# VinAIResearch/Point-Unet

Hardware: AMD Instinct MI355X
Metric: points_per_sec_forward (higher is better)
Workload: dtype f32

## Files before the change

point-unet_amd/csrc/att32_tile_walk.h:

```cpp
const int per_xcd = ((((a.n_total + 7) >> 3) + PPT - 1) / PPT) * PPT;
const int xcd = blockIdx.x & 7, slot = blockIdx.x >> 3, slots = gridDim.x >> 3;
const int t_end = min(a.n_total, (xcd + 1) * per_xcd);
const int t_first = xcd * per_xcd + (slot * TPW + tiw) * PPT, t_step = slots * TPW * PPT;
int n_pp[PPT], n_nl = 0;
float n_c[3], n_n[3];
const bool one_cloud = a.n_total == a.n_cloud;
auto cloud_base = [&](int row) { return one_cloud ? 0 : (row / a.n_cloud) * a.n_cloud; };
auto gstage = [&](int st, int t0n) {
    if (t0n >= t_end) return;
    if (st == 0) {
#pragma unroll
        for (int i = 0; i < PPT; ++i) {
            const int t = min(t0n + i, t_end - 1);
            n_pp[i] = a.order ? cloud_base(t) + a.order[t] : t;
        }
    } else if (st == 1) {
        const unsigned p = PPT == 2 ? (c32 >= KN ? n_pp[PPT - 1] : n_pp[0]) : n_pp[0];
        n_nl = a.idx[p * (unsigned)KN + (unsigned)(c32 & (KN - 1))];
        const float* cp = a.xyz + 3u * p;
        n_c[0] = cp[0]; n_c[1] = cp[1]; n_c[2] = cp[2];
    } else {
        const int p = PPT == 2 ? (c32 >= KN ? n_pp[PPT - 1] : n_pp[0]) : n_pp[0];
        n_nl += cloud_base(p);
        const float* np = a.xyz + 3u * (unsigned)n_nl;
        n_n[0] = np[0]; n_n[1] = np[1]; n_n[2] = np[2];
    }
};
gstage(0, t_first);
gstage(1, t_first);
gstage(2, t_first);
```

point-unet_amd/csrc/attpool32b.hip:

```cpp
#include "att32_tile.h"
#include "b3_ops.h"

namespace ps {

struct Att32bArgs : Att32ArgsT<uint4> {};

__device__ __forceinline__ B3Planes load_planes(const uint4* img, int slot, int lane)
{
    B3Planes r;
    r.p[0] = img[(slot * 3 + 0) * 64 + lane];
    r.p[1] = img[(slot * 3 + 1) * 64 + lane];
    r.p[2] = img[(slot * 3 + 2) * 64 + lane];
    return r;
}

template <int D, int STAGE, int KN, int WAVES>
__global__ __launch_bounds__(WAVES * 64) void att32b_kernel(Att32bArgs a)
{
    constexpr int H = D / 2, LDF = H + D, PITCH = H + 4, PPT = 32 / KN;
    constexpr int CBH = H / 32, CBD = D / 32, NQ = H / 16;
    constexpr int W1Q = CBH * 3 * 64, W2Q = STAGE == 2 ? CBH * NQ * 3 * 64 : 0, WBQ = CBD * NQ * 3 * 64;
    constexpr int TILE = 32 * PITCH;
    static_assert(H % 32 == 0 && (KN == 16 || KN == 32), "att32b: d_out >= 64, K in {16, 32}");

    extern __shared__ __attribute__((aligned(16))) float smem[];
    const int wave = __builtin_amdgcn_readfirstlane(threadIdx.x >> 6), lane = threadIdx.x & 63;
    const int hl = lane >> 5, c32 = lane & 31;
    uint4* Wq = reinterpret_cast<uint4*>(smem);
    constexpr int WTOT = (W1Q + W2Q + WBQ) * 4 + 2 * H;
    float* own = smem + WTOT + wave * (32 + TILE);
    int* NB = reinterpret_cast<int*>(own);
    float* T1 = own + 32;
    for (int i = threadIdx.x; i < W1Q; i += WAVES * 64) Wq[i] = a.w1[i];
    for (int i = threadIdx.x; i < W2Q; i += WAVES * 64) Wq[W1Q + i] = a.w2[i];
    for (int i = threadIdx.x; i < WBQ; i += WAVES * 64) Wq[W1Q + W2Q + i] = a.wb[i];
    float* bias = smem + (W1Q + W2Q + WBQ) * 4;
    for (int i = threadIdx.x; i < H; i += WAVES * 64) {
        bias[i] = a.b1[i];
        bias[H + i] = STAGE == 2 ? a.b2[i] : 0.f;
    }
    __syncthreads();
    const uint4 *w1 = Wq, *w2 = Wq + W1Q, *wb = Wq + W1Q + W2Q;
    const float *b1 = bias, *b2 = bias + H;

    constexpr int TPW = WAVES;
    const int tiw = wave;
#include "att32_tile_walk.h"
    for (int t0 = t_first; t0 < t_end; t0 += t_step) {
#include "att32_tile_row.h"
        const float ev[8] = ATT32_LOCSE_K16(enc);
        const B3Planes E = b3_split8<3>(ev);
        if (hl == 0) NB[c32] = nbr;
        gstage(0, t0 + t_step);
        wave_lds_sync();
        unsigned off[16];
        ATT32_ROW_OFFSETS(off, NB, LDF, (unsigned)c32 * 4u);
        const char* fgb = reinterpret_cast<const char*>(a.fg);
        f32x2 gq[2][8], v[2][8];
        auto gather = [&](int i, f32x2 (&gdst)[8], f32x2 (&vdst)[8]) {
            const int rel = i * 32 * 4;
#pragma unroll
            for (int r = 0; r < 16; ++r) gdst[r >> 1][r & 1] = *reinterpret_cast<const float*>(fgb + off[r] + (rel + H * 4));
            if (i * 32 < H) {
#pragma unroll
                for (int r = 0; r < 16; ++r) vdst[r >> 1][r & 1] = *reinterpret_cast<const float*>(fgb + off[r] + rel);
            }
        };
        gather(0, gq[0], v[0]);

        f32x16 f1[CBH];
#pragma unroll
        for (int cb = 0; cb < CBH; ++cb) {
            f32x16 acc;
            ATT32_BIAS_SEED(acc, b1, cb);
            acc = b3_mfma6<3>(load_planes(w1, cb, lane), E, acc);
#pragma unroll
            for (int r = 0; r < 16; ++r) f1[cb][r] = leaky02(acc[r]);
        }
        gstage(1, t0 + t_step);
        B3Planes P[NQ];
        auto split_block = [&](const f32x16& f, B3Planes& lo, B3Planes& hi) {
            const float x0[8] = {f[0], f[1], f[2], f[3], f[4], f[5], f[6], f[7]};
            const float x1[8] = {f[8], f[9], f[10], f[11], f[12], f[13], f[14], f[15]};
            lo = b3_split8<3>(x0);
            hi = b3_split8<3>(x1);
        };
        auto store_block = [&](const f32x16& f, int cb) {
            ATT32_STORE_BLOCK(T1 + c32 * PITCH, cb, , f);
        };
#pragma unroll
        for (int cb = 0; cb < CBH; ++cb) split_block(f1[cb], P[2 * cb], P[2 * cb + 1]);
        if constexpr (STAGE == 1) {
#pragma unroll
            for (int cb = 0; cb < CBH; ++cb) store_block(f1[cb], cb);
        } else {
            f32x16 f2[CBH];
#pragma unroll
            for (int cb = 0; cb < CBH; ++cb) {
                f32x16 acc;
                ATT32_BIAS_SEED(acc, b2, cb);
#pragma unroll
                for (int q = 0; q < NQ; ++q) acc = b3_mfma6<3>(load_planes(w2, cb * NQ + q, lane), P[q], acc);
#pragma unroll
                for (int r = 0; r < 16; ++r) f2[cb][r] = leaky02(acc[r]);
            }
#pragma unroll
            for (int cb = 0; cb < CBH; ++cb) {
                split_block(f2[cb], P[2 * cb], P[2 * cb + 1]);
                store_block(f2[cb], cb);
            }
        }
        wave_lds_sync();
        const float* TX = T1;

#pragma unroll
        for (int cb = 0; cb < CBD; ++cb) {
            if (cb + 1 < CBD) gather(cb + 1, gq[(cb + 1) & 1], v[(cb + 1) & 1]);
            if (cb == 0) gstage(2, t0 + t_step);
            f32x16 acc;
#pragma unroll
            for (int r = 0; r < 16; ++r) acc[r] = 0.f;
#pragma unroll
            for (int q = 0; q < NQ; ++q) acc = b3_mfma6<3>(P[q], load_planes(wb, cb * NQ + q, lane), acc);
            f32x2 (&vv)[8] = v[cb & 1];
            const f32x2 (&gs)[8] = gq[cb & 1];
#include "att32_tile_pool.h"
        }
        wave_lds_sync();
    }
}


template <int D, int STAGE, int KN, int WAVES>
__global__ __launch_bounds__(WAVES * 64) void att32s_kernel(Att32bArgs a)
{
    constexpr int H = D / 2, LDF = H + D, PITCH = H + 4, PPT = 32 / KN;
    constexpr int CBH = H / 32, CBD = D / 32, NQ = H / 16;
    constexpr int PLQ = NQ * 3 * 64;
    constexpr int NB_H = CBH / WAVES, NB_D = CBD / WAVES;
    static_assert(CBH % WAVES == 0 && NB_D == 2 && (KN == 16 || KN == 32), "att32s: two score blocks per wave");

    extern __shared__ __attribute__((aligned(16))) float smem[];
    const int wave = threadIdx.x >> 6, lane = threadIdx.x & 63;
    const int hl = lane >> 5, c32 = lane & 31;
    int* NB = reinterpret_cast<int*>(smem);
    uint4* PA = reinterpret_cast<uint4*>(smem + 32);
    uint4* PB = STAGE == 2 ? PA + PLQ : PA;
    float* TX = reinterpret_cast<float*>(PB + PLQ);

    constexpr int TPW = 1;
    const int tiw = 0;
#include "att32_tile_walk.h"
    auto seed = [&](const float* b, int cb) {
        f32x16 acc;
        ATT32_BIAS_SEED(acc, b, cb);
        return acc;
    };
    auto emit_block = [&](const f32x16& acc, int cb, uint4* planes, bool values) {
        float x0[8], x1[8];
#pragma unroll
        for (int r = 0; r < 8; ++r) { x0[r] = leaky02(acc[r]); x1[r] = leaky02(acc[8 + r]); }
        const B3Planes lo = b3_split8<3>(x0), hi = b3_split8<3>(x1);
#pragma unroll
        for (int pl = 0; pl < 3; ++pl) {
            planes[((2 * cb) * 3 + pl) * 64 + lane] = lo.p[pl];
            planes[((2 * cb + 1) * 3 + pl) * 64 + lane] = hi.p[pl];
        }
        if (values) {
#pragma unroll
            for (int g4 = 0; g4 < 4; ++g4) {
                const float* x = g4 < 2 ? x0 + 4 * g4 : x1 + 4 * (g4 - 2);
                *reinterpret_cast<float4*>(TX + c32 * PITCH + cb * 32 + g4 * 8 + hl * 4) = make_float4(x[0], x[1], x[2], x[3]);
            }
        }
    };
    static_assert(NB_H == 1, "att32s: one transposed block per wave");
    const B3Planes W1 = load_planes(a.w1, wave, lane);
    const f32x16 seed1 = seed(a.b1, wave);
    constexpr int PD = D >= 512 ? 4 : 2;
    constexpr int PD2 = STAGE == 2 ? (D >= 512 ? 4 : 8) : 1;
    const int cbA = wave, cbB = wave + WAVES;
    for (int t0 = t_first; t0 < t_end; t0 += t_step) {
#include "att32_tile_row.h"
        const float ev[8] = ATT32_LOCSE_K16(enc);
        const B3Planes E = b3_split8<3>(ev);
        if (hl == 0 && wave == 0) NB[c32] = nbr;
        gstage(0, t0 + t_step);
        B3Planes ring[PD2], rA[PD], rB[PD];
        if constexpr (STAGE == 2) {
#pragma unroll
            for (int q = 0; q < PD2; ++q) ring[q] = load_planes(a.w2, wave * NQ + q, lane);
        } else {
#pragma unroll
            for (int q = 0; q < PD; ++q) {
                rA[q] = load_planes(a.wb, cbA * NQ + q, lane);
                rB[q] = load_planes(a.wb, cbB * NQ + q, lane);
            }
        }

        emit_block(b3_mfma6<3>(W1, E, seed1), wave, PA, STAGE == 1);
        __syncthreads();
        gstage(1, t0 + t_step);
        unsigned off[16];
        ATT32_ROW_OFFSETS(off, NB, LDF, (unsigned)(wave * 32 + c32) * 4u);
        const char* fgb = reinterpret_cast<const char*>(a.fg);
        if constexpr (STAGE == 2) {
            const int cb = wave;
            f32x16 acc = seed(a.b2, cb);
#pragma unroll 1
            for (int q0 = 0; q0 + PD2 < NQ; q0 += PD2) {
#pragma unroll
                for (int j = 0; j < PD2; ++j) {
                    acc = b3_mfma6<3>(ring[j], load_planes(PA, q0 + j, lane), acc);
                    ring[j] = load_planes(a.w2, cb * NQ + q0 + j + PD2, lane);
                }
            }
#pragma unroll
            for (int j = 0; j < PD2; ++j) acc = b3_mfma6<3>(ring[j], load_planes(PA, NQ - PD2 + j, lane), acc);
#pragma unroll
            for (int q = 0; q < PD; ++q) {
                rA[q] = load_planes(a.wb, cbA * NQ + q, lane);
                rB[q] = load_planes(a.wb, cbB * NQ + q, lane);
            }
            emit_block(acc, cb, PB, true);
            __syncthreads();
        }
        gstage(2, t0 + t_step);

        f32x16 accA, accB;
#pragma unroll
        for (int r = 0; r < 16; ++r) { accA[r] = 0.f; accB[r] = 0.f; }
        f32x2 gq[2][8], v[2][8];
        {
#pragma unroll 1
            for (int q0 = 0; q0 + PD < NQ; q0 += PD) {
#pragma unroll
                for (int j = 0; j < PD; ++j) {
                    const B3Planes x = load_planes(PB, q0 + j, lane);
                    accA = b3_mfma6<3>(x, rA[j], accA);
                    accB = b3_mfma6<3>(x, rB[j], accB);
                    rA[j] = load_planes(a.wb, cbA * NQ + q0 + j + PD, lane);
                    rB[j] = load_planes(a.wb, cbB * NQ + q0 + j + PD, lane);
                }
            }
#pragma unroll
            for (int i = 0; i < 2; ++i)
#pragma unroll
                for (int r = 0; r < 16; ++r) gq[i][r >> 1][r & 1] = *reinterpret_cast<const float*>(fgb + off[r] + (i * WAVES * 32 * 4 + H * 4));
#pragma unroll
            for (int j = 0; j < PD; ++j) {
                const B3Planes x = load_planes(PB, NQ - PD + j, lane);
                accA = b3_mfma6<3>(x, rA[j], accA);
                accB = b3_mfma6<3>(x, rB[j], accB);
            }
        }
#pragma unroll
        for (int r = 0; r < 16; ++r) v[0][r >> 1][r & 1] = *reinterpret_cast<const float*>(fgb + off[r]);
#pragma unroll
        for (int ii = 0; ii < 2; ++ii) {
            const int i = 1 - ii;
            const int cb = wave + i * WAVES;
            const f32x16& acc = i == 0 ? accA : accB;
            f32x2 (&vv)[8] = v[i];
            const f32x2 (&gs)[8] = gq[i];
#include "att32_tile_pool.h"
        }
        __syncthreads();
    }
}

static inline int kmap(int q, int g, int j)
{
    const int r = 8 * (q & 1) + j;
    return 32 * (q >> 1) + (r & 3) + 8 * (r >> 2) + 4 * g;
}

void pack_b3(const float* W, int cin, int cout, uint16_t* out)
{
    const int nq = cin / 16, cbs = cout / 32;
    for (int cb = 0; cb < cbs; ++cb)
        for (int q = 0; q < nq; ++q)
            for (int pl = 0; pl < 3; ++pl)
                for (int l = 0; l < 64; ++l)
                    for (int j = 0; j < 8; ++j)
                        out[(((((size_t)cb * nq + q) * 3 + pl) * 64 + l) * 8) + j] = b3_piece_of(W[(size_t)kmap(q, l >> 5, j) * cout + 32 * cb + (l & 31)], pl);
}

void pack_b3_locse(const float* W1, int cout, uint16_t* out)
{
    const int cbs = cout / 32;
    for (int cb = 0; cb < cbs; ++cb)
        for (int pl = 0; pl < 3; ++pl)
            for (int l = 0; l < 64; ++l)
                for (int j = 0; j < 8; ++j) {
                    const int k = 8 * (l >> 5) + j;
                    out[((((size_t)cb * 3 + pl) * 64 + l) * 8) + j] = k < 10 ? b3_piece_of(W1[(size_t)k * cout + 32 * cb + (l & 31)], pl) : (uint16_t)0;
                }
}

template <int D, int STAGE, int KN>
static int launch_att32b(ps_context* c, const Att32bArgs& a)
{
    constexpr int H = D / 2, PITCH = H + 4, TILE = 32 * PITCH;
    constexpr int CBH = H / 32, CBD = D / 32, NQ = H / 16;
    constexpr int WAVES = D == 128 ? 8 : (STAGE == 1 ? 16 : 12);
    constexpr int PER_CU = 1;
    constexpr size_t planes = (size_t)(CBH + (STAGE == 2 ? CBH * NQ : 0) + CBD * NQ) * 3 * 64 * 16;
    constexpr size_t smem = planes + sizeof(float) * (2 * H + (size_t)WAVES * (32 + TILE));
    static_assert(smem <= 160 * 1024, "att32b: weights + tiles exceed the LDS");
    auto kern = att32b_kernel<D, STAGE, KN, WAVES>;
    PS_HIP(hipFuncSetAttribute(reinterpret_cast<const void*>(kern), hipFuncAttributeMaxDynamicSharedMemorySize, (int)smem));
    const int tiles = ceil_div(a.n_total, 32 / KN);
    const int blocks = (std::min(ceil_div(tiles, WAVES), 256 * PER_CU) + 7) & ~7;
    hipLaunchKernelGGL(kern, dim3(blocks), dim3(WAVES * 64), smem, c->stream, a);
    PS_HIP(hipGetLastError());
    return PS_OK;
}

template <int D, int STAGE, int KN>
static int launch_att32s(ps_context* c, const Att32bArgs& a)
{
    constexpr int H = D / 2, PITCH = H + 4, NQ = H / 16;
    constexpr int WAVES = D / 64;
    constexpr size_t smem = sizeof(float) * 32 + (size_t)(STAGE == 2 ? 2 : 1) * NQ * 3 * 64 * 16 + sizeof(float) * 32 * PITCH;
    static_assert(smem <= 160 * 1024, "att32s: planes + value tile exceed the LDS");
    auto kern = att32s_kernel<D, STAGE, KN, WAVES>;
    if (smem > 48 * 1024) PS_HIP(hipFuncSetAttribute(reinterpret_cast<const void*>(kern), hipFuncAttributeMaxDynamicSharedMemorySize, (int)smem));
    const int tiles = ceil_div(a.n_total, 32 / KN);
    const int blocks = (std::min(tiles, 256 * 16) + 7) & ~7;
    hipLaunchKernelGGL(kern, dim3(blocks), dim3(WAVES * 64), smem, c->stream, a);
    PS_HIP(hipGetLastError());
    return PS_OK;
}

bool att_pool32b_fits(const AttStage& s)
{
    return att_pool32_fits(s) && s.p32->w1b && (s.d == 64 || s.d == 128 || s.d == 256 || s.d == 512);
}

int att_pool32b_stage(ps_context* c, const AttStage& s)
{
    if (s.n_total <= 0) return PS_OK;
    const Att32bArgs a = att32_args<Att32bArgs>(s, s.p32->w1b, s.p32->w2b, s.p32->wb1b, s.p32->wb2b);
    if (s.d == 64) return att32_stage_k(s, [&](auto stage, auto k) { return launch_att32b<64, stage(), k()>(c, a); });
    if (s.d == 128) return att32_stage_k(s, [&](auto stage, auto k) { return launch_att32b<128, stage(), k()>(c, a); });
    if (s.d == 256) return att32_stage_k(s, [&](auto stage, auto k) { return launch_att32s<256, stage(), k()>(c, a); });
    return att32_stage_k(s, [&](auto stage, auto k) { return launch_att32s<512, stage(), k()>(c, a); });
}

}
```

point-unet_amd/csrc/debug_hooks.h:

```cpp
#ifndef POINTSEG_DEBUG_H
#define POINTSEG_DEBUG_H
#include "../../include/pointseg.h"
#ifdef __cplusplus
extern "C" {
#endif
int ps_debug_knn_host(const float* support, const float* queries, int64_t B, int64_t n_support,
                      int64_t n_queries, int64_t K, int32_t* out_idx);
int ps_debug_kdtree_host(const float* support, int64_t n, int32_t* vind, int32_t* nodes, float* pts,
                         int32_t* root_depth, float* bbox);
int ps_debug_kdtree_device(ps_context* ctx, const float* support, int64_t n, int32_t* vind, int32_t* nodes,
                           float* pts, int32_t* root_depth, float* bbox);
#define PS_DEBUG_KDTREE_STATS 22
int ps_debug_kdtree_device_set(ps_context* ctx, const float* support, const int32_t* n, int64_t T, const int32_t* want_copy, int32_t* vind,
                               int32_t* nodes, float* pts, int32_t* fat, int32_t* root_depth, float* bbox, float* copy, int32_t* stats);
int ps_debug_pack_weights(const float* W, int cin, int cout, int ntb, float* out);
int ps_debug_pack_b3(const float* W, int cin, int cout, uint16_t* out);
int ps_debug_gemm32(ps_context* ctx, int split_bf16, const float* x1, int ld1, int c1, const int32_t* g1, const float* x2, int ld2, int c2,
                    const int32_t* g2, int gm, int gn, const float* W, const float* bias, int64_t R, int cout, int leaky, float* y, int ldy);
int ps_debug_gemm32_plan(ps_context* ctx, int split_bf16, int64_t R, int cin, int cout, int* out4);

typedef struct ps_debug_chain_layer {
    const float* W;
    const float* bias;
    int cin, cout, leaky;
    float* y;
    int ldy;
    const float* extra;
    int ld_extra, c_extra;
    const int32_t* extra_gather;
} ps_debug_chain_layer;
typedef struct ps_debug_chain_desc {
    int n_layers;
    ps_debug_chain_layer layer[4];
    const float* x1; const int32_t* g1; int ld1, c1, g1m, g1n;
    const float* x2; const int32_t* g2; int ld2, c2, g2m, g2n;
    int64_t R;
} ps_debug_chain_desc;
int ps_debug_chain(ps_context* ctx, const ps_debug_chain_desc* d, int form);
int ps_debug_chain_plan(const ps_debug_chain_desc* d, int* out4);
int ps_debug_set_regchain_b3(ps_context* ctx, int on);
int ps_debug_set_att_lane(ps_context* ctx, int on);
int ps_debug_att_stage(ps_randla* net, int level, int stage, int form, const float* xyz, const int32_t* idx, const int32_t* order, const float* fg,
                       int64_t n_total, int64_t n_cloud, float* agg);
int ps_debug_att_form(ps_randla* net, int level, int stage, int k, int64_t n_total);
int ps_debug_att_lane_pass_points(void);

int ps_debug_set_tuning(ps_context* ctx, const char* field, double value);
int ps_debug_get_tuning(ps_context* ctx, const char* field, double* value);
int ps_debug_tuning_fields(char* buf, int cap);
int ps_debug_volume_sample_args_size(void);

int64_t ps_debug_scan_words(int64_t n);
int64_t ps_debug_sort_words(int64_t n);
int ps_debug_scan_launches(int64_t n);
int ps_debug_sort_launches(int64_t n, int bits);
int ps_debug_scan_u32(ps_context* ctx, const uint32_t* in, uint32_t* out, int64_t n, uint32_t* work);
int ps_debug_sort_pairs(ps_context* ctx, int key_bytes, void* k0, void* k1, uint32_t* v0, uint32_t* v1, int64_t n, int bits, uint32_t* work,
                        int* which_out);
int ps_debug_reduce_partials(ps_context* ctx, int form, const void* part, int n_part, int nv, int n0, void* out0, void* out1);

#ifdef __cplusplus
}
#endif
#endif
```

point-unet_amd/csrc/debug_hooks.hip:

```cpp
#include "common.h"

#include <cstring>
#include <vector>
#include "kdtree_build.h"
#include "kdtree_host.h"
#include "rowgemm.h"
#include "attpool.h"
#include "debug_hooks.h"
#include "randla_net.h"
#include "reduce_partials.h"
#include "sortscan.h"

using namespace ps;

extern "C" int ps_debug_volume_sample_args_size(void) { return (int)sizeof(ps_volume_sample_args); }

extern "C" int ps_debug_pack_weights(const float* W, int cin, int cout, int ntb, float* out)
{
    PS_CHECK(W && out && (ntb == 1 || ntb == 2 || ntb == 4), "ps_debug_pack_weights: bad argument");
    pack_weights(W, cin, cout, ntb, out);
    return PS_OK;
}

extern "C" int ps_debug_pack_b3(const float* W, int cin, int cout, uint16_t* out)
{
    PS_CHECK(W && out && cin > 0 && cin % 32 == 0 && cout > 0 && cout % 32 == 0, "ps_debug_pack_b3: bad argument");
    pack_b3(W, cin, cout, out);
    return PS_OK;
}

extern "C" int ps_debug_gemm32(ps_context* c, int split_bf16, const float* x1, int ld1, int c1, const int32_t* g1, const float* x2, int ld2, int c2,
                               const int32_t* g2, int gm, int gn, const float* W, const float* bias, int64_t R, int cout, int leaky, float* y, int ldy)
{
    PS_CHECK(c && x1 && W && bias && y && R >= 0 && c1 > 0 && c2 >= 0 && cout > 0, "ps_debug_gemm32: bad argument");
    PS_HIP(hipSetDevice(c->device));
    const int cin = c1 + c2;
    PS_CHECK(cin % (split_bf16 ? 16 : 8) == 0 && cout % 32 == 0, "ps_debug_gemm32: cin %% %d and cout %% 32 must be 0", split_bf16 ? 16 : 8);
    std::vector<float> img((size_t)cin * cout * (split_bf16 ? 3 : 2) / 2);
    if (split_bf16) pack_p32b(W, cin, cout, reinterpret_cast<uint16_t*>(img.data()));
    else pack_p32(W, cin, cout, img.data());
    float *d_img = nullptr, *d_bias = nullptr;
    PS_HIP(hipMalloc(reinterpret_cast<void**>(&d_img), img.size() * sizeof(float)));
    PS_HIP(hipMalloc(reinterpret_cast<void**>(&d_bias), sizeof(float) * (size_t)cout));
    PS_HIP(hipMemcpyAsync(d_img, img.data(), img.size() * sizeof(float), hipMemcpyHostToDevice, c->stream));
    PS_HIP(hipMemcpyAsync(d_bias, bias, sizeof(float) * (size_t)cout, hipMemcpyHostToDevice, c->stream));
    PackedLinear L;
    L.cin = cin; L.cout = cout; L.leaky = leaky; L.bias = d_bias;
    if (split_bf16) L.w32b = d_img; else L.w32 = d_img;
    RowSrc s1, s2;
    s1.x = x1; s1.ld = ld1; s1.c = c1; s1.gather = g1; s1.gm = g1 ? gm : 0; s1.gn = g1 ? gn : 0;
    s2.x = x2; s2.ld = ld2; s2.c = c2; s2.gather = g2; s2.gm = g2 ? gm : 0; s2.gn = g2 ? gn : 0;
    int rc = PS_EINVAL;
    if (split_bf16 ? gemm32b_fits(L, s1, s2, R, ldy) : gemm32_fits(L, s1, s2, R, ldy))
        rc = split_bf16 ? gemm32b(c, L, s1, s2, R, y, ldy) : gemm32(c, L, s1, s2, R, y, ldy);
    else
        set_error("ps_debug_gemm32: the shape does not fit the kernel");
    (void)hipStreamSynchronize(c->stream);
    (void)hipFree(d_img);
    (void)hipFree(d_bias);
    return rc;
}

extern "C" int ps_debug_gemm32_plan(ps_context* c, int split_bf16, int64_t R, int cin, int cout, int* out4)
{
    PS_CHECK(c && out4 && R >= 1 && cin > 0 && cout > 0 && cin % (split_bf16 ? 16 : 8) == 0 && cout % 32 == 0, "ps_debug_gemm32_plan: bad argument");
    const Gemm32Plan p = split_bf16 ? gemm32b_plan(c->tune, R, cin, cout) : gemm32_plan(c->tune, R, cin, cout);
    out4[0] = p.rw;
    out4[1] = p.cw;
    out4[2] = p.sk;
    out4[3] = p.pd;
    return PS_OK;
}

namespace {

struct ChainBuild {
    PackedLinear L[kChainMaxSteps];
    ChainStep steps[kChainMaxSteps];
    RowSrc s1, s2;
    int n = 0;
};

int chain_describe(const ps_debug_chain_desc* d, ChainBuild& b, const float* image)
{
    PS_CHECK(d && d->n_layers >= 1 && d->n_layers <= kChainMaxSteps, "ps_debug_chain: 1..%d layers", kChainMaxSteps);
    PS_CHECK(d->R >= 0 && d->c1 > 0 && d->c2 >= 0 && d->ld1 >= d->c1 && (d->c2 == 0 || d->ld2 >= d->c2), "ps_debug_chain: bad row sources");
    b.n = d->n_layers;
    b.s1.x = d->x1; b.s1.gather = d->g1; b.s1.ld = d->ld1; b.s1.c = d->c1; b.s1.gm = d->g1 ? d->g1m : 0; b.s1.gn = d->g1 ? d->g1n : 0;
    if (d->c2) {
        b.s2.x = d->x2; b.s2.gather = d->g2; b.s2.ld = d->ld2; b.s2.c = d->c2; b.s2.gm = d->g2 ? d->g2m : 0; b.s2.gn = d->g2 ? d->g2n : 0;
    }
    for (int i = 0; i < b.n; ++i) {
        const ps_debug_chain_layer& y = d->layer[i];
        PS_CHECK(y.cin > 0 && y.cout > 0 && y.cin <= 4096 && y.cout <= 4096, "ps_debug_chain: layer %d: bad channel counts", i);
        PS_CHECK(!y.y || y.ldy >= y.cout, "ps_debug_chain: layer %d: ldy below cout", i);
        PS_CHECK(!y.extra || (i > 0 && y.c_extra > 0 && y.ld_extra >= y.c_extra), "ps_debug_chain: layer %d: bad extra source", i);
        PackedLinear& L = b.L[i];
        L = PackedLinear();
        L.cin = y.cin; L.cout = y.cout; L.leaky = y.leaky;
        L.ks = (y.cin + 3) / 4;
        L.ntb = choose_ntb(y.cout);
        L.cblocks = (y.cout + 16 * L.ntb - 1) / (16 * L.ntb);
        L.wp = image; L.bias = image;
        ChainStep& st = b.steps[i];
        st = ChainStep();
        st.L = &L; st.y = y.y; st.ldy = y.ldy;
        if (y.extra) {
            st.extra.x = y.extra; st.extra.ld = y.ld_extra; st.extra.c = y.c_extra; st.extra.gather = y.extra_gather;
        }
    }
    return PS_OK;
}

}

extern "C" int ps_debug_chain_plan(const ps_debug_chain_desc* d, int* out4)
{
    PS_CHECK(d && out4 && d->R >= 1, "ps_debug_chain_plan: bad argument");
    static const float nothing = 0.f;
    ChainBuild b;
    PS_TRY(chain_describe(d, b, &nothing));
    const ChainPlan p = rowchain_plan(b.steps, b.n, b.s1, b.s2, d->R);
    out4[0] = p.form;
    out4[1] = p.form ? p.blocks : 0;
    out4[2] = p.form ? (int)p.lds_bytes : 0;
    out4[3] = p.fast_in;
    return PS_OK;
}

extern "C" int ps_debug_chain(ps_context* c, const ps_debug_chain_desc* d, int form)
{
    PS_CHECK(c && d && form >= 0 && form <= 3, "ps_debug_chain: bad argument");
    ChainBuild b;
    PS_TRY(chain_describe(d, b, nullptr));
    PS_CHECK(d->x1 && (d->c2 == 0 || d->x2), "ps_debug_chain: NULL row source");
    for (int i = 0; i < b.n; ++i) PS_CHECK(d->layer[i].W, "ps_debug_chain: layer %d has no weights", i);
    if (form == 3) {
        int cur = d->c1 + d->c2;
        for (int i = 0; i < b.n; ++i) {
            const ps_debug_chain_layer& y = d->layer[i];
            PS_CHECK(!(y.extra && y.extra_gather), "ps_debug_chain: layer %d: the extra rows of a chain are plain rows", i);
            cur += y.extra ? y.c_extra : 0;
            PS_CHECK(cur == y.cin, "ps_debug_chain: layer %d expects %d channels, the chain gives %d", i, y.cin, cur);
            cur = y.cout;
        }
    }
    if (d->R == 0) return PS_OK;
    PS_HIP(hipSetDevice(c->device));
    std::vector<float> host;
    size_t wp_off[kChainMaxSteps], b_off[kChainMaxSteps], wq_off[kChainMaxSteps], tmp_off[kChainMaxSteps];
    auto grow = [&](size_t floats) {
        const size_t off = (host.size() + 63) & ~size_t(63);
        host.resize(off + floats);
        return off;
    };
    for (int i = 0; i < b.n; ++i) {
        const ps_debug_chain_layer& y = d->layer[i];
        PackedLinear& L = b.L[i];
        wp_off[i] = grow(L.packed_floats());
        pack_weights(y.W, y.cin, y.cout, L.ntb, host.data() + wp_off[i]);
        b_off[i] = grow((size_t)L.cout_pad());
        for (int k = 0; k < L.cout_pad(); ++k) host[b_off[i] + k] = (y.bias && k < y.cout) ? y.bias[k] : 0.f;
        wq_off[i] = 0;
        if (y.cin % 16 == 0) {
            wq_off[i] = grow(L.kperm_floats());
            pack_weights_kperm(y.W, y.cin, y.cout, L.ntb, host.data() + wq_off[i]);
        }
    }
    size_t total = (host.size() + 63) & ~size_t(63);
    for (int i = 0; i < b.n; ++i) {
        tmp_off[i] = total;
        if (form == 3 && !d->layer[i].y) total += ((size_t)d->R * d->layer[i].cout + 63) & ~size_t(63);
    }
    float* dev = nullptr;
    PS_HIP(hipMalloc(reinterpret_cast<void**>(&dev), total * sizeof(float)));
    int rc = PS_OK;
    if (hipMemcpyAsync(dev, host.data(), host.size() * sizeof(float), hipMemcpyHostToDevice, c->stream) != hipSuccess) {
        set_error("ps_debug_chain: upload failed");
        rc = PS_EHIP;
    }
    for (int i = 0; i < b.n; ++i) {
        b.L[i].wp = dev + wp_off[i];
        b.L[i].bias = dev + b_off[i];
        b.L[i].wq = wq_off[i] ? dev + wq_off[i] : nullptr;
    }
    if (rc == PS_OK) {
        if (form == 0) {
            ChainCache cache;
            if (rowchain_fits(b.steps, b.n, b.s1, b.s2)) rc = rowchain(c, b.steps, b.n, b.s1, b.s2, d->R, &cache);
            else { set_error("ps_debug_chain: the chain fits neither chain kernel (channels above %d, mismatched, or a gathered extra)", kChainMaxC); rc = PS_EINVAL; }
            (void)hipStreamSynchronize(c->stream);
            cache.clear();
        } else if (form == 1) {
            if (regchain_fits(b.steps, b.n, b.s1, b.s2)) rc = regchain(c, b.steps, b.n, b.s1, b.s2, d->R, nullptr);
            else { set_error("ps_debug_chain: not one of regchain's compiled chain shapes"); rc = PS_EINVAL; }
        } else if (form == 2) {
            if (rowchain_lds_plan(b.steps, b.n, b.s1, b.s2, d->R).form == 2) rc = rowchain_lds(c, b.steps, b.n, b.s1, b.s2, d->R);
            else { set_error("ps_debug_chain: the chain does not fit the LDS-staged kernel (channels above %d, mismatched, or a gathered extra)", kChainMaxC); rc = PS_EINVAL; }
        } else {
            RowSrc in1 = b.s1, in2 = b.s2;
            for (int i = 0; i < b.n && rc == PS_OK; ++i) {
                const ChainStep& st = b.steps[i];
                if (i > 0) {
                    in2 = RowSrc();
                    if (st.extra.x) in2 = st.extra;
                }
                float* out = st.y ? st.y : dev + tmp_off[i];
                const int ldo = st.y ? st.ldy : b.L[i].cout;
                rc = rowgemm(c, b.L[i], in1, in2, d->R, out, ldo);
                in1 = RowSrc();
                in1.x = out; in1.ld = ldo; in1.c = b.L[i].cout;
            }
        }
    }
    (void)hipStreamSynchronize(c->stream);
    (void)hipFree(dev);
    return rc;
}

extern "C" int ps_debug_set_regchain_b3(ps_context* c, int on)
{
    PS_CHECK(c && (on == 0 || on == 1), "ps_debug_set_regchain_b3: bad argument");
    c->regchain_b3 = on != 0;
    return PS_OK;
}

extern "C" int ps_debug_set_att_lane(ps_context* c, int on)
{
    PS_CHECK(c && (on == 0 || on == 1), "ps_debug_set_att_lane: bad argument");
    c->att_lane = on != 0;
    return PS_OK;
}

extern "C" int ps_debug_att_stage(ps_randla* net, int level, int stage, int form, const float* xyz, const int32_t* idx, const int32_t* order,
                                  const float* fg, int64_t n_total, int64_t n_cloud, float* agg)
{
    PS_CHECK(net && xyz && idx && fg && agg, "ps_debug_att_stage: NULL argument");
    PS_CHECK(net->have_weights, "ps_debug_att_stage: weights not set");
    PS_CHECK(level >= 0 && level < net->cfg.num_layers && (stage == 1 || stage == 2) && form >= 0 && form <= 4, "ps_debug_att_stage: bad level / stage / form");
    PS_CHECK(n_total >= 0 && n_cloud >= 1 && n_total % n_cloud == 0, "ps_debug_att_stage: n_total must be a whole number of clouds");
    ps_context* c = net->ctx;
    PS_HIP(hipSetDevice(c->device));
    const EncLevel& e = net->enc[level];
    const int d = e.d, h = d / 2;
    const bool use_g = d >= 64;
    AttStage s;
    s.xyz = xyz; s.idx = idx; s.order = order; s.fg = fg; s.lfa1 = &e.lfa1; s.agg = agg;
    s.n_total = n_total; s.n_cloud = n_cloud; s.d = d; s.k = net->cfg.k_n; s.ldf = use_g ? h + d : h;
    s.p32 = e.has_p32 ? &e.p32 : nullptr;
    s.lfa2 = stage == 2 ? &e.lfa2 : nullptr;
    s.wbot = use_g ? (stage == 1 ? &e.bot1 : &e.bot2) : nullptr;
    s.wfull = use_g ? nullptr : (stage == 1 ? &e.full1 : &e.full2);
    s.lane = stage == 1 ? e.lane1 : e.lane2;
    int rc = PS_EINVAL;
    if (form == 4) rc = att_lane_stage(c, s);
    else if (form == 0) rc = att_pool_stage(c, s);
    else if (form == 1 && att_pool32b_fits(s)) rc = att_pool32b_stage(c, s);
    else if (form == 2 && att_pool32_fits(s)) rc = att_pool32_stage(c, s);
    else if (form == 3) rc = att_pool16_stage(c, s);
    else set_error("ps_debug_att_stage: the level (d = %d, %lld rows) does not fit the 32x32 form %d", d, (long long)n_total, form);
    (void)hipStreamSynchronize(c->stream);
    return rc;
}

extern "C" int ps_debug_att_form(ps_randla* net, int level, int stage, int k, int64_t n_total)
{
    if (!net || !net->have_weights || level < 0 || level >= net->cfg.num_layers || (stage != 1 && stage != 2) || k < 1 || n_total < 0) {
        set_error("ps_debug_att_form: bad argument");
        return -1;
    }
    const EncLevel& e = net->enc[level];
    const int d = e.d, h = d / 2;
    const bool use_g = d >= 64;
    AttStage s;
    s.lfa1 = &e.lfa1; s.lfa2 = stage == 2 ? &e.lfa2 : nullptr;
    s.wbot = use_g ? (stage == 1 ? &e.bot1 : &e.bot2) : nullptr;
    s.wfull = use_g ? nullptr : (stage == 1 ? &e.full1 : &e.full2);
    s.lane = stage == 1 ? e.lane1 : e.lane2;
    s.p32 = e.has_p32 ? &e.p32 : nullptr;
    s.n_total = n_total; s.n_cloud = n_total; s.d = d; s.k = k; s.ldf = use_g ? h + d : h;
    return att_pool_form(net->ctx, s);
}

extern "C" int ps_debug_att_lane_pass_points(void) { return att_lane_pass_points(); }

static bool is_bool(double v) { return v == 0 || v == 1; }
static bool is_int_in(double v, double lo, double hi) { return v >= lo && v <= hi && v == (double)(int64_t)v; }

#define PS_TUNING_FIELDS(X)                                                \
    X(gemm32b_min_flops, v >= 0 && v <= 1e300)                             \
    X(gemm32b_rw, v == 0 || v == 1 || v == 2)                              \
    X(gemm32b_cw, v == 0 || v == 1 || v == 2)                              \
    X(gemm32_no_sk8, is_bool(v))                                           \
    X(att64_gemm, is_bool(v))                                              \
    X(att64_occ, v == 0 || v == 1 || v == 2)                               \
    X(att_no_split, is_bool(v))                                            \
    X(wgrad_b3_min_rows, is_int_in(v, 0, (double)(1ll << 40)))             \
    X(gemm_b3_min_rows, is_int_in(v, 0, (double)(1ll << 40)))              \
    X(wgrad_wgs, is_int_in(v, 64, 4096))                                   \
    X(bn_slice, is_bool(v))                                                \
    X(inv_bucket, is_bool(v))                                              \
    X(inv_tile, v == 4096 || v == 6144 || v == 8192)                       \
    X(gather_reduce_ordered, is_bool(v))                                   \
    X(maxpool_bwd_ordered, is_bool(v))                                     \
    X(train_act_bf16, is_bool(v))                                          \
    X(train_att_gemm_split, v == -1 || v == 0 || v == 1)                   \
    X(train_att_gemm, is_bool(v))                                          \
    X(train_att128_fwd_gemm, is_bool(v))                                   \
    X(train_fuse_residual, is_bool(v))                                     \
    X(train_merge_syncbn, is_bool(v))                                      \
    X(convbn_max_c, is_int_in(v, 0, 4096))                                 \
    X(convbn_rect_max, is_int_in(v, 0, (double)(1 << 30)))                 \
    X(wgrad_debug, is_bool(v))

extern "C" int ps_debug_set_tuning(ps_context* c, const char* field, double v)
{
    PS_CHECK(c && field, "ps_debug_set_tuning: NULL argument");
#define PS_SET(f, ok)                                                                                 \
    if (std::strcmp(field, #f) == 0) {                                                                \
        PS_CHECK(ok, "ps_debug_set_tuning: %g is not a value %s is compiled for", v, #f);             \
        c->tune.f = static_cast<decltype(c->tune.f)>(v);                                              \
        return PS_OK;                                                                                 \
    }
    PS_TUNING_FIELDS(PS_SET)
#undef PS_SET
    PS_CHECK(false, "ps_debug_set_tuning: no knob named '%s'", field);
}

extern "C" int ps_debug_get_tuning(ps_context* c, const char* field, double* out)
{
    PS_CHECK(c && field && out, "ps_debug_get_tuning: NULL argument");
#define PS_GET(f, ok)                               \
    if (std::strcmp(field, #f) == 0) {              \
        *out = static_cast<double>(c->tune.f);      \
        return PS_OK;                               \
    }
    PS_TUNING_FIELDS(PS_GET)
#undef PS_GET
    PS_CHECK(false, "ps_debug_get_tuning: no knob named '%s'", field);
}

extern "C" int ps_debug_tuning_fields(char* buf, int cap)
{
    static const char names[] =
#define PS_NAME(f, ok) #f "\n"
        PS_TUNING_FIELDS(PS_NAME)
#undef PS_NAME
        ;
    PS_CHECK(buf && cap >= (int)sizeof(names), "ps_debug_tuning_fields: need %d bytes", (int)sizeof(names));
    std::memcpy(buf, names, sizeof(names));
    return PS_OK;
}

extern "C" int ps_debug_kdtree_device(ps_context* c, const float* support, int64_t n, int32_t* vind, int32_t* nodes, float* pts,
                                      int32_t* root_depth, float* bbox)
{
    PS_CHECK(c && support && vind && nodes && pts && root_depth && bbox && n >= 1, "ps_debug_kdtree_device: bad argument");
    PS_HIP(hipSetDevice(c->device));
    PS_TRY(c->stage_in.reserve(sizeof(float) * 3 * (size_t)n));
    PS_HIP(hipMemcpyAsync(c->stage_in.p, support, sizeof(float) * 3 * (size_t)n, hipMemcpyHostToDevice, c->stream));
    TreeSetPlan plan;
    plan.add((int32_t)n);
    for (int pass = 0; pass < 2; ++pass) {
        c->knn_arena.begin(pass == 0);
        plan.carve(c->knn_arena);
        if (pass == 0) PS_TRY(c->knn_arena.buf.reserve(c->knn_arena.off));
    }
    plan.src[0] = c->stage_in.as<float>();
    PS_TRY(build_trees(c, plan));
    int32_t flag[kBuildFlagWords] = {};
    PS_HIP(hipMemcpyAsync(flag, plan.d_flags, sizeof(flag), hipMemcpyDeviceToHost, c->stream));
    PS_HIP(hipStreamSynchronize(c->stream));
    PS_CHECK(flag[kFlagQueueOverflow] == 0, "ps_debug_kdtree_device: builder queue overflow");
    TreeMeta m;
    PS_HIP(hipMemcpyAsync(nodes, plan.d_nodes[0], sizeof(int4) * 2 * (size_t)n, hipMemcpyDeviceToHost, c->stream));
    PS_HIP(hipMemcpyAsync(pts, plan.d_pts[0], sizeof(float4) * (size_t)n, hipMemcpyDeviceToHost, c->stream));
    PS_HIP(hipMemcpyAsync(&m, plan.d_meta, sizeof(TreeMeta), hipMemcpyDeviceToHost, c->stream));
    PS_HIP(hipStreamSynchronize(c->stream));
    for (int64_t i = 0; i < n; ++i) std::memcpy(&vind[i], &pts[4 * i + 3], 4);
    root_depth[0] = m.root;
    root_depth[1] = m.depth;
    for (int a = 0; a < 3; ++a) {
        bbox[a] = m.lo[a];
        bbox[3 + a] = m.hi[a];
    }
    return PS_OK;
}

extern "C" int ps_debug_kdtree_device_set(ps_context* c, const float* support, const int32_t* n, int64_t T, const int32_t* want_copy, int32_t* vind,
                                          int32_t* nodes, float* pts, int32_t* fat, int32_t* root_depth, float* bbox, float* copy, int32_t* stats)
{
    PS_CHECK(c && support && n && T >= 1 && vind && nodes && pts && fat && root_depth && bbox && stats, "ps_debug_kdtree_device_set: bad argument");
    size_t tot = 0, tot_copy = 0;
    for (int64_t i = 0; i < T; ++i) {
        PS_CHECK(n[i] >= 1, "ps_debug_kdtree_device_set: tree %lld has %d points", (long long)i, n[i]);
        tot += (size_t)n[i];
        if (want_copy && want_copy[i]) tot_copy += (size_t)n[i];
    }
    PS_CHECK(tot_copy == 0 || copy, "ps_debug_kdtree_device_set: want_copy without a copy buffer");
    PS_HIP(hipSetDevice(c->device));
    PS_TRY(c->stage_in.reserve(sizeof(float) * 3 * tot));
    PS_HIP(hipMemcpyAsync(c->stage_in.p, support, sizeof(float) * 3 * tot, hipMemcpyHostToDevice, c->stream));
    TreeSetPlan plan;
    for (int64_t i = 0; i < T; ++i) plan.add(n[i]);
    float* d_copy = nullptr;
    for (int pass = 0; pass < 2; ++pass) {
        c->knn_arena.begin(pass == 0);
        plan.carve(c->knn_arena);
        d_copy = c->knn_arena.take<float>(3 * tot_copy + 1);
        if (pass == 0) PS_TRY(c->knn_arena.buf.reserve(c->knn_arena.off));
    }
    plan.copy_dst.assign((size_t)T, nullptr);
    {
        size_t off = 0, off_copy = 0;
        for (int64_t i = 0; i < T; ++i) {
            plan.src[i] = c->stage_in.as<float>() + 3 * off;
            off += (size_t)n[i];
            if (want_copy && want_copy[i]) {
                plan.copy_dst[i] = d_copy + 3 * off_copy;
                off_copy += (size_t)n[i];
            }
        }
    }
    PS_TRY(build_trees(c, plan));
    BuildCounters bc;
    PS_TRY(read_build_counters(c, plan, &bc));
    int32_t flag[kBuildFlagWords] = {};
    PS_HIP(hipMemcpyAsync(flag, plan.d_flags, sizeof(flag), hipMemcpyDeviceToHost, c->stream));
    std::vector<TreeMeta> meta((size_t)T);
    PS_HIP(hipMemcpyAsync(meta.data(), plan.d_meta, sizeof(TreeMeta) * (size_t)T, hipMemcpyDeviceToHost, c->stream));
    {
        size_t off = 0;
        for (int64_t i = 0; i < T; ++i) {
            const size_t ni = (size_t)n[i];
            PS_HIP(hipMemcpyAsync(nodes + 4 * 2 * off, plan.d_nodes[i], sizeof(int4) * 2 * ni, hipMemcpyDeviceToHost, c->stream));
            PS_HIP(hipMemcpyAsync(fat + 4 * 6 * off, plan.d_fat[i], sizeof(int4) * 6 * ni, hipMemcpyDeviceToHost, c->stream));
            PS_HIP(hipMemcpyAsync(pts + 4 * off, plan.d_pts[i], sizeof(float4) * ni, hipMemcpyDeviceToHost, c->stream));
            off += ni;
        }
    }
    if (tot_copy) PS_HIP(hipMemcpyAsync(copy, d_copy, sizeof(float) * 3 * tot_copy, hipMemcpyDeviceToHost, c->stream));
    PS_HIP(hipStreamSynchronize(c->stream));
    for (size_t i = 0; i < tot; ++i) std::memcpy(&vind[i], &pts[4 * i + 3], 4);
    for (int64_t i = 0; i < T; ++i) {
        root_depth[2 * i] = meta[(size_t)i].root;
        root_depth[2 * i + 1] = meta[(size_t)i].depth;
        for (int a = 0; a < 3; ++a) {
            bbox[6 * i + a] = meta[(size_t)i].lo[a];
            bbox[6 * i + 3 + a] = meta[(size_t)i].hi[a];
        }
    }
    static_assert(PS_DEBUG_KDTREE_STATS == 6 + 2 * kBuildCounterLevels, "stats layout (debug_hooks.h)");
    stats[0] = bc.chunked_levels;
    for (int l = 0; l < kBuildCounterLevels; ++l) {
        stats[1 + l] = bc.ntasks[l];
        stats[1 + kBuildCounterLevels + l] = bc.nchunks[l];
    }
    stats[1 + 2 * kBuildCounterLevels] = bc.straggler_tasks;
    stats[2 + 2 * kBuildCounterLevels] = bc.mid_pushed;
    stats[3 + 2 * kBuildCounterLevels] = bc.small_pushed;
    stats[4 + 2 * kBuildCounterLevels] = flag[kFlagStackOverflow];
    stats[5 + 2 * kBuildCounterLevels] = flag[kFlagQueueOverflow];
    return PS_OK;
}

extern "C" int64_t ps_debug_scan_words(int64_t n) { return n < 0 ? -1 : (int64_t)scan_workspace_words((size_t)n); }
extern "C" int64_t ps_debug_sort_words(int64_t n) { return n < 0 ? -1 : (int64_t)sort_workspace_words((size_t)n); }
extern "C" int ps_debug_scan_launches(int64_t n) { return n < 0 ? -1 : scan_launches((size_t)n); }
extern "C" int ps_debug_sort_launches(int64_t n, int bits) { return n < 0 || bits < 1 || bits > 64 ? -1 : radix_sort_pairs_launches((size_t)n, bits); }

extern "C" int ps_debug_scan_u32(ps_context* c, const uint32_t* in, uint32_t* out, int64_t n, uint32_t* work)
{
    PS_CHECK(c && in && out && work && n >= 0, "ps_debug_scan_u32: bad argument");
    PS_HIP(hipSetDevice(c->device));
    exclusive_scan_u32(c->stream, in, out, (size_t)n, work);
    PS_HIP(hipGetLastError());
    PS_HIP(hipStreamSynchronize(c->stream));
    return PS_OK;
}

extern "C" int ps_debug_sort_pairs(ps_context* c, int key_bytes, void* k0, void* k1, uint32_t* v0, uint32_t* v1, int64_t n, int bits, uint32_t* work,
                                   int* which_out)
{
    PS_CHECK(c && k0 && k1 && v0 && v1 && work && which_out && n >= 0, "ps_debug_sort_pairs: bad argument");
    PS_CHECK(key_bytes == 4 || key_bytes == 8, "ps_debug_sort_pairs: key_bytes must be 4 or 8");
    PS_CHECK(bits >= 1 && bits <= 8 * key_bytes, "ps_debug_sort_pairs: bits must be 1..%d", 8 * key_bytes);
    PS_HIP(hipSetDevice(c->device));
    *which_out = key_bytes == 4
                     ? radix_sort_pairs_u32(c->stream, static_cast<unsigned*>(k0), static_cast<unsigned*>(k1), v0, v1, (size_t)n, bits, work)
                     : radix_sort_pairs_u64(c->stream, static_cast<unsigned long long*>(k0), static_cast<unsigned long long*>(k1), v0, v1, (size_t)n,
                                            bits, work);
    PS_HIP(hipGetLastError());
    PS_HIP(hipStreamSynchronize(c->stream));
    return PS_OK;
}

extern "C" int ps_debug_reduce_partials(ps_context* c, int form, const void* part, int n_part, int nv, int n0, void* out0, void* out1)
{
    PS_CHECK(c && part && out0 && n_part >= 0 && nv >= 0 && form >= 0 && form <= 3, "ps_debug_reduce_partials: bad argument");
    PS_CHECK(form < 2 || (out1 && n0 >= 0 && n0 <= nv), "ps_debug_reduce_partials: forms 2 and 3 need out1 and 0 <= n0 <= nv");
    PS_HIP(hipSetDevice(c->device));
    if (nv == 0) return PS_OK;
    const dim3 grid((unsigned)((nv + 15) / 16)), block(256);
    switch (form) {
    case 0:
        hipLaunchKernelGGL(reduce_partials_kernel<float>, grid, block, 0, c->stream, static_cast<const float*>(part), n_part, nv, static_cast<float*>(out0));
        break;
    case 1:
        hipLaunchKernelGGL(reduce_partials_kernel<double>, grid, block, 0, c->stream, static_cast<const double*>(part), n_part, nv,
                           static_cast<double*>(out0));
        break;
    case 2:
        hipLaunchKernelGGL((reduce_partials2_kernel<float>), grid, block, 0, c->stream, static_cast<const float*>(part), n_part, nv, n0,
                           static_cast<float*>(out0), static_cast<float*>(out1));
        break;
    default:
        hipLaunchKernelGGL((reduce_partials2_kernel<float, double>), grid, block, 0, c->stream, static_cast<const float*>(part), n_part, nv, n0,
                           static_cast<float*>(out0), static_cast<float*>(out1));
        break;
    }
    PS_HIP(hipGetLastError());
    PS_HIP(hipStreamSynchronize(c->stream));
    return PS_OK;
}
```

Before: 203.9 million.

## Interleave wave tile walk, batch weight staging loads, use buffer loads for gather

```diff
diff --git a/point-unet_amd/csrc/att32_tile_walk.h b/point-unet_amd/csrc/att32_tile_walk.h
--- a/point-unet_amd/csrc/att32_tile_walk.h
+++ b/point-unet_amd/csrc/att32_tile_walk.h
@@ -1,7 +1,7 @@
 const int per_xcd = ((((a.n_total + 7) >> 3) + PPT - 1) / PPT) * PPT;
 const int xcd = blockIdx.x & 7, slot = blockIdx.x >> 3, slots = gridDim.x >> 3;
 const int t_end = min(a.n_total, (xcd + 1) * per_xcd);
-const int t_first = xcd * per_xcd + (slot * TPW + tiw) * PPT, t_step = slots * TPW * PPT;
+const int t_first = xcd * per_xcd + (tiw * slots + slot) * PPT, t_step = slots * TPW * PPT;
 int n_pp[PPT], n_nl = 0;
 float n_c[3], n_n[3];
 const bool one_cloud = a.n_total == a.n_cloud;
diff --git a/point-unet_amd/csrc/attpool32b.hip b/point-unet_amd/csrc/attpool32b.hip
--- a/point-unet_amd/csrc/attpool32b.hip
+++ b/point-unet_amd/csrc/attpool32b.hip
@@ -4,6 +4,15 @@
 namespace ps {
 
 struct Att32bArgs : Att32ArgsT<uint4> {};
+
+__device__ __forceinline__ __amdgpu_buffer_rsrc_t fg_rsrc(const float* fg, unsigned bytes)
+{
+    return __builtin_amdgcn_make_buffer_rsrc(const_cast<float*>(fg), 0, (int)bytes, 0x00020000);
+}
+__device__ __forceinline__ float fg_load(__amdgpu_buffer_rsrc_t r, unsigned off)
+{
+    return __builtin_bit_cast(float, __builtin_amdgcn_raw_buffer_load_b32(r, (int)off, 0, 0));
+}
 
 __device__ __forceinline__ B3Planes load_planes(const uint4* img, int slot, int lane)
 {
@@ -12,6 +21,23 @@
     r.p[1] = img[(slot * 3 + 1) * 64 + lane];
     r.p[2] = img[(slot * 3 + 2) * 64 + lane];
     return r;
+}
+
+template <int N, int NT, int R>
+__device__ __forceinline__ void stage_load(uint4 (&r)[R], const uint4* __restrict__ src, int tid)
+{
+#pragma unroll
+    for (int j = 0; j * NT < N; ++j) r[j] = src[(j + 1) * NT <= N ? tid + j * NT : min(tid + j * NT, N - 1)];
+}
+template <int N, int NT, bool WHOLE, int R>
+__device__ __forceinline__ void stage_write(uint4* dst, const uint4 (&r)[R], int tid)
+{
+#pragma unroll
+    for (int j = 0; j * NT < N; ++j) {
+        if ((j + 1) * NT <= N) {
+            if (WHOLE) dst[tid + j * NT] = r[j];
+        } else if (!WHOLE && tid + j * NT < N) dst[tid + j * NT] = r[j];
+    }
 }
 
 template <int D, int STAGE, int KN, int WAVES>
@@ -31,9 +57,22 @@
     float* own = smem + WTOT + wave * (32 + TILE);
     int* NB = reinterpret_cast<int*>(own);
     float* T1 = own + 32;
-    for (int i = threadIdx.x; i < W1Q; i += WAVES * 64) Wq[i] = a.w1[i];
-    for (int i = threadIdx.x; i < W2Q; i += WAVES * 64) Wq[W1Q + i] = a.w2[i];
-    for (int i = threadIdx.x; i < WBQ; i += WAVES * 64) Wq[W1Q + W2Q + i] = a.wb[i];
+    {
+        constexpr int NT = WAVES * 64;
+        constexpr int N1 = (W1Q + NT - 1) / NT, N2 = (W2Q + NT - 1) / NT, NB3 = (WBQ + NT - 1) / NT;
+        static_assert(N1 + N2 + NB3 <= 12, "att32b: the staging loads of a thread are held in registers");
+        const int tid = threadIdx.x;
+        uint4 r1[N1], r2[N2 ? N2 : 1], rb[NB3];
+        stage_load<W1Q, NT>(r1, a.w1, tid);
+        stage_load<W2Q, NT>(r2, a.w2, tid);
+        stage_load<WBQ, NT>(rb, a.wb, tid);
+        stage_write<W1Q, NT, true>(Wq, r1, tid);
+        stage_write<W2Q, NT, true>(Wq + W1Q, r2, tid);
+        stage_write<WBQ, NT, true>(Wq + W1Q + W2Q, rb, tid);
+        stage_write<W1Q, NT, false>(Wq, r1, tid);
+        stage_write<W2Q, NT, false>(Wq + W1Q, r2, tid);
+        stage_write<WBQ, NT, false>(Wq + W1Q + W2Q, rb, tid);
+    }
     float* bias = smem + (W1Q + W2Q + WBQ) * 4;
     for (int i = threadIdx.x; i < H; i += WAVES * 64) {
         bias[i] = a.b1[i];
@@ -45,6 +84,7 @@
 
     constexpr int TPW = WAVES;
     const int tiw = wave;
+    const __amdgpu_buffer_rsrc_t fgr = fg_rsrc(a.fg, (unsigned)a.n_total * (unsigned)(LDF * 4));
 #include "att32_tile_walk.h"
     for (int t0 = t_first; t0 < t_end; t0 += t_step) {
 #include "att32_tile_row.h"
@@ -55,15 +95,14 @@
         wave_lds_sync();
         unsigned off[16];
         ATT32_ROW_OFFSETS(off, NB, LDF, (unsigned)c32 * 4u);
-        const char* fgb = reinterpret_cast<const char*>(a.fg);
         f32x2 gq[2][8], v[2][8];
         auto gather = [&](int i, f32x2 (&gdst)[8], f32x2 (&vdst)[8]) {
             const int rel = i * 32 * 4;
 #pragma unroll
-            for (int r = 0; r < 16; ++r) gdst[r >> 1][r & 1] = *reinterpret_cast<const float*>(fgb + off[r] + (rel + H * 4));
+            for (int r = 0; r < 16; ++r) gdst[r >> 1][r & 1] = fg_load(fgr, off[r] + (rel + H * 4));
             if (i * 32 < H) {
 #pragma unroll
-                for (int r = 0; r < 16; ++r) vdst[r >> 1][r & 1] = *reinterpret_cast<const float*>(fgb + off[r] + rel);
+                for (int r = 0; r < 16; ++r) vdst[r >> 1][r & 1] = fg_load(fgr, off[r] + rel);
             }
         };
         gather(0, gq[0], v[0]);
diff --git a/point-unet_amd/csrc/debug_hooks.h b/point-unet_amd/csrc/debug_hooks.h
--- a/point-unet_amd/csrc/debug_hooks.h
+++ b/point-unet_amd/csrc/debug_hooks.h
@@ -15,6 +15,7 @@
                                int32_t* nodes, float* pts, int32_t* fat, int32_t* root_depth, float* bbox, float* copy, int32_t* stats);
 int ps_debug_pack_weights(const float* W, int cin, int cout, int ntb, float* out);
 int ps_debug_pack_b3(const float* W, int cin, int cout, uint16_t* out);
+int ps_debug_pack_b3_device(ps_context* ctx, const float* W, int cin, int cout, void* out);
 int ps_debug_gemm32(ps_context* ctx, int split_bf16, const float* x1, int ld1, int c1, const int32_t* g1, const float* x2, int ld2, int c2,
                     const int32_t* g2, int gm, int gn, const float* W, const float* bias, int64_t R, int cout, int leaky, float* y, int ldy);
 int ps_debug_gemm32_plan(ps_context* ctx, int split_bf16, int64_t R, int cin, int cout, int* out4);
diff --git a/point-unet_amd/csrc/debug_hooks.hip b/point-unet_amd/csrc/debug_hooks.hip
--- a/point-unet_amd/csrc/debug_hooks.hip
+++ b/point-unet_amd/csrc/debug_hooks.hip
@@ -27,6 +27,21 @@
     PS_CHECK(W && out && cin > 0 && cin % 32 == 0 && cout > 0 && cout % 32 == 0, "ps_debug_pack_b3: bad argument");
     pack_b3(W, cin, cout, out);
     return PS_OK;
+}
+
+extern "C" int ps_debug_pack_b3_device(ps_context* c, const float* W, int cin, int cout, void* out)
+{
+    PS_CHECK(c && W && out && cin > 0 && cin % 32 == 0 && cout > 0 && cout % 32 == 0, "ps_debug_pack_b3_device: bad argument");
+    PS_HIP(hipSetDevice(c->device));
+    PackJob j{};
+    j.w = W; j.sk = cout; j.sn = 1; j.kind = 5; j.cin = cin; j.cout = cout; j.out = out;
+    j.total = (int64_t)(cin / 16) * (cout / 32) * 64;
+    PackJob* table = nullptr;
+    PS_HIP(hipMalloc(reinterpret_cast<void**>(&table), sizeof(PackJob)));
+    int rc = hipMemcpy(table, &j, sizeof(PackJob), hipMemcpyHostToDevice) == hipSuccess ? pack_batch_b3(c, table, 1) : PS_EINVAL;
+    (void)hipStreamSynchronize(c->stream);
+    (void)hipFree(table);
+    return rc;
 }
 
 extern "C" int ps_debug_gemm32(ps_context* c, int split_bf16, const float* x1, int ld1, int c1, const int32_t* g1, const float* x2, int ld2, int c2,
```

Result: faster. 206.2 million, median of 6 (+1.2%).
